# alasdairforsythe/tokenmonster

Hardware: AMD Instinct MI355X
Metric: GB/s raw UTF-8 tokenized, englishcode-32000 vocab (higher is better)
Workload: dtype u8; 1 GPU; englishcode-32000-consistent vocabulary shape (synthetic, 32000 ids / 54181 index records), 1024 MiB raw synthetic mixed text per GPU in 300327 documents; end to end: input = RAW UTF-8 resident in HBM, normalized (NFD+capcode) on the GPU inside the timed step, output = uint32 ids + offsets in HBM; raw_bytes_per_gpu=1073743404, normalized_bytes_per_gpu=1145560274, missing=0, parallelism=documents sharded by rank, no collective, rccl_ranks=0

## Files before the change

tokenmonster_amd/csrc/tm_norm.hip:

```cpp
#include <hip/hip_runtime.h>

#include <algorithm>
#include <chrono>
#include <cstring>
#include <mutex>
#include <thread>
#include <vector>

#include "tm_pipeline.h"
#include "tm_build.h"
#include "tm_norm_masks.h"

using namespace tmh;

namespace tmh {

constexpr int PIECE = 1024, PMARGIN = 68, PLDS = PIECE + 2 * PMARGIN;
constexpr uint32_t PS_WHOLE = 1u, PS_LEADU_SHIFT = 1, PS_LEADTL = 8u, PS_TRAILU_SHIFT = 5, PS_FIRSTBLOCK = 128u, PS_FIRSTL = 256u, PS_BAD = 512u;

__device__ __forceinline__ uint32_t ncls_ascii(uint32_t c, bool lower_all) {
  if (c - 'a' < 26u) return NC_L;
  if (c - 'A' < 26u) return lower_all ? NC_L : NC_U;
  if (c - '0' < 10u) return NC_N;
  if (c == '\'') return NC_AP;
// ... 232 lines not shown
  if (np_dev) npieces = min(npieces, np_dev[0]);
  __shared__ PieceLds s_l[4];
  __shared__ uint8_t s_cls[128];
  __shared__ TabLds s_tab;
  if (threadIdx.x < 128) s_cls[threadIdx.x] = (uint8_t)ncls_ascii(threadIdx.x, lower_all != 0);
  const NmTabs tabs = stage_tabs(s_tab, two);
  __syncthreads();
  const int lane = threadIdx.x & 63, wv = threadIdx.x >> 6;
  const uint64_t k = (uint64_t)blockIdx.x * 4 + wv;
  if (k >= npieces) return;
  PieceLds& L = s_l[wv];
  const uint32_t d = piece_doc[k];
  if (MODE != 3 && need_host[d]) { if (MODE != 1 && lane == 0) piece_len[k] = 0; return; }
  const uint64_t rb = rbegin[d], re = rend[d], pb = rb + (k - doc_piece_start[d]) * PIECE;
  const int m = norm_load_piece(L, raw, rb, re, pb, lane, s_cls, &s_tab, two);
  uint8_t* dst = MODE == 1 ? out + piece_off[k] : (MODE >= 2 ? out + k * (uint64_t)SLAB : nullptr);
  if (capcode != 2 || MODE == 3) {
    if (MODE != 1 && lane == 0) piece_len[k] = (uint32_t)m;
    bool bad = false;
    if (WRITE) for (int i = lane; i < m; i += 64) {
      const int x = PMARGIN + i;
      if (MODE == 3) bad |= L.f[x] == NF_BAD;
      uint32_t b = L.raw[x], y = 0, m3 = 0;
      if (lower_all && b - 'A' < 26u) b |= 0x20u;
      const uint32_t bm1 = L.raw[x - 1];
      if (nm_two_lead(b)) (void)nm_two_out(nm_two_get(tabs, nm_two_index(b, L.raw[x + 1])), false, false, false, &b, &y, &m3);
      else if (nm_cont_byte(b) && nm_two_lead(bm1)) (void)nm_two_out(nm_two_get(tabs, nm_two_index(bm1, b)), true, false, false, &b, &y, &m3);
      dst[i] = (uint8_t)b;
    }
    if (MODE == 3 && __any(bad) && lane == 0) need_host[d] = 1;
    return;
  }
  const uint32_t carry = piece_carry[k];
  const unsigned long long below = (1ull << lane) - 1ull;
  {
    uint32_t carry_ua = (carry >> 2) & 3u;
    bool carry_tl = (carry >> 4) & 1u;
    for (int c = (m - 1) / 64; c >= 0; c--) {
      const int i = c * 64 + lane;
      const bool in = i < m;
      const uint32_t fl = in ? L.f[PMARGIN + i] : 0u, cls = fl & NF_CLASS;
      const unsigned long long V = __ballot(in), mB = __ballot(in && nblock(cls)), mU = __ballot(in && cls == NC_U), mL = __ballot(in && cls == NC_L);
      const unsigned long long above = lane == 63 ? 0ull : (~0ull << (lane + 1));
      const unsigned long long stop = V & ~mB & above;
      uint32_t ua;
      bool tl;
      if (stop != 0) {
        const int e = __ffsll((long long)stop) - 1;
        ua = (uint32_t)__popcll(mU & above & ((1ull << e) - 1ull));
        tl = (mL >> e) & 1ull;
      } else {
        ua = (uint32_t)__popcll(mU & above) + carry_ua;
        tl = carry_tl;
      }
      ua = min(ua, 2u);
      if (in && nblock(cls)) L.f[PMARGIN + i] = (uint8_t)(fl | (tl ? NF_TERML : 0u) | (ua << NF_UA_SHIFT));
      const uint32_t ua0 = __shfl(ua, 0), cls0 = __shfl(cls, 0);
      const bool tl0 = __shfl((int)tl, 0) != 0;
      if (nblock(cls0)) { carry_ua = min(ua0 + (cls0 == NC_U ? 1u : 0u), 2u); carry_tl = tl0; }
      else { carry_ua = 0; carry_tl = cls0 == NC_L; }
    }
  }
  const bool next_tl = (carry >> 4) & 1u;
  __builtin_amdgcn_wave_barrier();
  __builtin_amdgcn_s_waitcnt(0);
  uint32_t carry_ub = carry & 3u;
  uint32_t pos = 0;
  for (int c = 0; c * 64 < m; c++) {
    const int i = c * 64 + lane, x = PMARGIN + i;
    const bool in = i < m;
    const uint32_t fl = in ? L.f[x] : 0u, cls = fl & NF_CLASS;
    const unsigned long long mB = __ballot(in && nblock(cls)), mU = __ballot(in && cls == NC_U);
    const unsigned long long gap = ~mB & below;
    uint32_t ub;
    if (gap != 0) {
      const int s = 64 - __clzll((long long)gap);
      ub = (uint32_t)__popcll(mU & below & ~((1ull << s) - 1ull));
    } else ub = (uint32_t)__popcll(mU & below) + carry_ub;
    ub = min(ub, 2u);
    {
      const uint32_t ub63 = __shfl(ub, 63), cls63 = __shfl(cls, 63);
      carry_ub = nblock(cls63) ? min(ub63 + (cls63 == NC_U ? 1u : 0u), 2u) : 0u;
    }
    uint32_t o0 = 0, o1 = 0, o2 = 0, o3 = 0, len = 0;
    if (in) {
      const uint32_t b = L.raw[x];
      const uint32_t fm1 = L.f[x - 1], P = fm1 & NF_CLASS;
      uint32_t P2 = NC_O;
      if (P == NC_AP) P2 = L.f[(fm1 & NF_CONT) ? x - 4 : x - 2] & NF_CLASS;
      const bool inword = ub >= 1;
      const bool tl = (fl & NF_TERML) != 0;
      const uint32_t code = nm_lut_entry(nm_lut_index((fl & NF_CONT) ? (uint32_t)NC_O : cls, P, P2, inword ? 1u : 0u, tl ? 1u : 0u), lower_all != 0);
      len = (code & 3u) + 1u;
      o0 = 'D'; o1 = code >> 8; o2 = ' ';
      o3 = b | ((code & 4u) << 3);
      if (cls == NC_SP) {
        const bool last = i + 1 == m;
        const uint32_t fp1 = L.f[x + 1];
        if ((fp1 & NF_CLASS) == NC_U && fp1 != NF_BAD && !(fp1 & NF_CONT)) o3 = (last ? next_tl : (fp1 & NF_TERML) != 0) ? 'C' : 'W';
      }
      const uint32_t bm1 = L.raw[x - 1];
      const bool lead2 = nm_two_lead(b), cont2 = nm_cont_byte(b) && nm_two_lead(bm1);
      if (lead2 || cont2) {
        const NmTwo e = nm_two_get(tabs, lead2 ? nm_two_index(b, L.raw[x + 1]) : nm_two_index(bm1, b));
        uint32_t y = 0, m3 = 0;
        const uint32_t extra = nm_two_out(e, cont2, (code & 4u) != 0, true, &o3, &y, &m3);
        if (extra >= 1u) { len = 1u + extra; o2 = y; o1 = m3; }
      }
      uint32_t hrole, hcp;
      if ((tabs.misc & NM_MISC_HANGUL) && fl != NF_BAD && nm_hangul_role(b, bm1, L.raw[x - 2], L.raw[x + 1], L.raw[x + 2], &hrole, &hcp)) len = nm_hangul_out(hcp, hrole, &o1, &o2, &o3);
      uint32_t lrole, lidx;
      if ((tabs.misc & NM_MISC_LEA) && fl != NF_BAD && nm_lea_role(b, bm1, L.raw[x - 2], L.raw[x + 1], L.raw[x + 2], &lrole, &lidx) && (tabs.lea[lidx].a & NT_OK)) {
        const NmLea le = tabs.lea[lidx];
        if (lrole == 0u) o3 = (code & 4u) ? ((le.a >> 16) & 0xFFu) : ((le.a >> 8) & 0xFFu);
        else if (lrole == 1u) { len = 2u; o2 = le.b & 0xFFu; o3 = (le.b >> 8) & 0xFFu; }
        else if (((le.a >> 24) & 3u) == 2u) { len = 2u; o2 = (le.b >> 16) & 0xFFu; o3 = le.b >> 24; }
        else len = 0u;
      }
      uint32_t krole, kidx;
      if ((tabs.misc & NM_MISC_KANA) && fl != NF_BAD && nm_kana_role(b, bm1, L.raw[x - 2], L.raw[x + 1], L.raw[x + 2], &krole, &kidx) && (nm_kana_tab(tabs)[kidx] & NK_OK))
        len = nm_kana_out(nm_kana_tab(tabs)[kidx], krole, &o1, &o2, &o3);
      uint32_t drole, dcp;
      if ((tabs.misc & NM_MISC_DEC3) && fl != NF_BAD && nm_three_role(b, bm1, L.raw[x - 2], L.raw[x + 1], L.raw[x + 2], &drole, &dcp) && (nm_dec3(tabs, dcp) & ND_OK))
        len = nm_dec3_out(tabs, nm_dec3(tabs, dcp), drole, &o1, &o2, &o3);
    }
    uint32_t incl = len;
#pragma unroll
    for (uint32_t q = 1; q <= 4; q++) {
      const unsigned long long bq = __ballot(len >= q);
      incl = __builtin_amdgcn_mbcnt_hi((uint32_t)(bq >> 32), __builtin_amdgcn_mbcnt_lo((uint32_t)bq, incl));
    }
    if (WRITE && in && (MODE == 1 || pos + incl <= (uint32_t)SLAB)) {
      uint8_t* w = dst + pos + (incl - len);
      if (len == 4) { w[0] = (uint8_t)o0; w[1] = (uint8_t)o1; w[2] = (uint8_t)o2; w[3] = (uint8_t)o3; }
      else if (len == 3) { w[0] = (uint8_t)o1; w[1] = (uint8_t)o2; w[2] = (uint8_t)o3; }
      else if (len == 2) { w[0] = (uint8_t)o2; w[1] = (uint8_t)o3; }
      else if (len == 1) w[0] = (uint8_t)o3;
    }
    pos += __shfl(incl, 63);
  }
  if (MODE != 1 && lane == 0) {
    piece_len[k] = pos;
    if (MODE == 2 && pos > (uint32_t)SLAB) atomicAdd(overflow, 1ull);
  }
}

struct PieceLds2 { uint8_t raw[PLDS]; uint8_t f[PLDS]; uint8_t chg[32]; alignas(16) uint8_t out[2 * PIECE + 64]; };

__device__ const NmLut g_norm_lut = nm_make_lut();

#ifndef TM_NORM_UNROLL
#define TM_NORM_UNROLL 2
#endif
template <bool CARRY>
__global__ __launch_bounds__(256) void k_norm_emit2(const uint8_t* __restrict__ raw, const uint64_t* __restrict__ rbegin,
                                                    const uint64_t* __restrict__ rend, const uint32_t* __restrict__ piece_doc,
                                                    const uint64_t* __restrict__ doc_piece_start, uint64_t npieces, uint32_t lower_all,
                                                    const uint8_t* __restrict__ piece_carry, uint8_t* __restrict__ need_host,
                                                    uint32_t* __restrict__ piece_len, uint8_t* __restrict__ slab,
                                                    unsigned long long* __restrict__ overflow, const NmTwo* __restrict__ two,
                                                    const uint64_t* __restrict__ np_dev) {
  constexpr int SLAB2 = 2 * PIECE, NCH = PIECE / 64;
  if (np_dev) npieces = min(npieces, np_dev[0]);
  __shared__ PieceLds2 s_l[4];
  __shared__ uint8_t s_cls[128];
  __shared__ TabLds s_tab;
  const NmTabs tabs = stage_tabs(s_tab, two);
  alignas(16) __shared__ uint16_t s_lut[NM_LUT_SIZE];
  static_assert(NM_LUT_SIZE * sizeof(uint16_t) == 256 * sizeof(uint4), "one 16-byte load per thread stages the rule table");
  if (threadIdx.x < 128) s_cls[threadIdx.x] = (uint8_t)ncls_ascii(threadIdx.x, lower_all != 0);
  reinterpret_cast<uint4*>(s_lut)[threadIdx.x] = reinterpret_cast<const uint4*>(g_norm_lut.e[lower_all ? 1 : 0])[threadIdx.x];
  __syncthreads();
  const int lane = threadIdx.x & 63, wv = __builtin_amdgcn_readfirstlane((int)(threadIdx.x >> 6));
  PieceLds2& L = s_l[wv];
#pragma unroll 1
  for (uint64_t k = (uint64_t)blockIdx.x * 4 + wv; k < npieces; k += (uint64_t)gridDim.x * 4) {
  const uint32_t d = piece_doc[k];
  if (CARRY && need_host[d]) { if (lane == 0) piece_len[k] = 0; continue; }
  const uint64_t rb = rbegin[d], re = rend[d], pb = rb + (k - doc_piece_start[d]) * PIECE;
  const int m = __builtin_amdgcn_readfirstlane(norm_load_piece(L, raw, rb, re, pb, lane, s_cls, &s_tab, two));
  const uint32_t carry = CARRY ? __builtin_amdgcn_readfirstlane((uint32_t)piece_carry[k]) : 0u;
  const int nch = (m + 63) >> 6;
  const uint8_t* fl0 = L.f + PMARGIN + lane;
  unsigned long long w_seed = (carry & 3u) ? 1ull : 0ull;
  const unsigned long long t0_beyond = CARRY ? (unsigned long long)((carry >> 4) & 1u) : 0ull;
  if (!CARRY) {
    const uint32_t fb = fl0[-64], fa = m == PIECE ? (uint32_t)fl0[64 * NCH] : 0u;
    uint64_t w_in;
    const bool known = nm_margin_carries(__ballot((fb & NF_BLOCK) != 0), __ballot((fb & NF_CLASS) == NC_U), __ballot((fa & NF_BLOCK) != 0), &w_in);
    if (!known && lane == 0) atomicAdd(overflow + 1, 1ull);
    w_seed = w_in;
  }
  typedef TM_LDS_SPACE uint8_t lds_u8;
  const uint32_t out0 = TM_LDS_ADDR(L.out);
  const uint32_t dump = out0 + (uint32_t)SLAB2 + (uint32_t)lane;
  const uint32_t lim = out0 + (uint32_t)SLAB2;
  unsigned long long w = w_seed, badm = 0ull;
  uint32_t posabs = out0;
  bool over = false;
  uint32_t chC = 'C', chW = 'W', chSP = ' ', chD = 'D';
  TM_KEEP_IN_VGPRS4(chC, chW, chSP, chD);
  const uint8_t* fc = fl0;
  const uint8_t* rc = L.raw + PMARGIN + lane;
  uint32_t fl = fc[0];
  unsigned long long Bcur = __ballot((fl & NF_BLOCK) != 0), Lcur = __ballot((fl & NF_CLASS) == NC_L), Ucur = __ballot((fl & NF_CLASS) == NC_U);
  int c = 0;
  auto chunk = [&]() __attribute__((always_inline)) {
    const uint32_t fnext = fc[64];
    const unsigned long long Bn = __ballot((fnext & NF_BLOCK) != 0), Ln = __ballot((fnext & NF_CLASS) == NC_L), Un = __ballot((fnext & NF_CLASS) == NC_U);
    unsigned long long t0n = Ln >> __builtin_ctzll(~Bn | (1ull << 63));
    if (__builtin_expect(Bn == ~0ull, 0)) {
      t0n = t0_beyond;
#pragma unroll 1
      for (int j = c + 2; j <= NCH; j++) {
        const uint32_t fj = fl0[64 * j];
        const unsigned long long Bj = __ballot((fj & NF_BLOCK) != 0), Lj = __ballot((fj & NF_CLASS) == NC_L);
        if (Bj != ~0ull) { t0n = nm_t0(Bj, Lj, 0ull); break; }
      }
    }
    const unsigned long long TXc = nm_tx(Bcur, Lcur, t0n);
    const uint32_t fp = fc[-1], f2 = fc[-2], f4 = fc[-4];
    const uint32_t b = rc[0];
    uint64_t w_out, spC, spW;
    if (!CARRY) badm |= __ballot(fl == NF_BAD);
    const unsigned long long W = nm_inword(Bcur, Ucur, ~0ull, w, &w_out);
    nm_space_markers(__ballot((fl & NF_CLASS) == NC_SP), Ucur, Un, ~0ull, TXc, t0n, &spC, &spW);
    w = w_out;
    const uint32_t p2 = (fp & NF_CONT) ? f4 : f2;
    uint32_t idx = ((fl & NF_CONT) ? (uint32_t)NC_O : (fl & 7u)) | ((fp & 7u) << 3) | ((p2 & 7u) << 6);
    idx = sel_mask(W, idx | 512u, idx);
    idx = sel_mask(TXc, idx | 1024u, idx);
    const uint32_t code = s_lut[idx];
    uint32_t len1 = code & 3u;
    uint32_t o3 = b | ((code & 4u) << 3);
    o3 = sel_mask(spC, chC, o3);
    o3 = sel_mask(spW, chW, o3);
    uint32_t ysp = chSP, m3 = code >> 8;
    unsigned long long E = ~0ull;
    uint32_t below = posabs + (uint32_t)lane, n = len1 + 1u;
    if (__ballot(b >= 0x80u) != 0ull && __builtin_amdgcn_readfirstlane((int)L.chg[c]) != 0) {
      if (b >= 0x80u) {
        const HighOut h = emit_high_byte(rc, fl, code, HighOut{o3, ysp, m3, len1}, &s_tab, two);
        o3 = h.o3; ysp = h.ysp; m3 = h.m3; len1 = h.len1;
      }
      E = ~__ballot(len1 == 0xFFu);
      len1 = len1 == 0xFFu ? 0u : len1;
      n = sel_mask(E, len1 + 1u, 0u);
      below = mbcnt64(E, posabs);
    }
    const unsigned long long ge2 = __ballot(len1 >= 1u), ge3 = __ballot(len1 >= 2u), ge4 = __ballot(len1 >= 3u);
    const uint32_t first = mbcnt64(ge4, mbcnt64(ge3, mbcnt64(ge2, below)));
    const uint32_t last = first + len1;
    const uint32_t end = read_lane(first + n, 63);
    if (end <= lim) {
      *TM_LDS_PTR(lds_u8, sel_mask(E, last, dump)) = (uint8_t)o3;
      *TM_LDS_PTR(lds_u8, sel_mask(ge2, last - 1u, dump)) = (uint8_t)ysp;
      *TM_LDS_PTR(lds_u8, sel_mask(ge3, last - 2u, dump)) = (uint8_t)m3;
      *TM_LDS_PTR(lds_u8, sel_mask(ge4, first, dump)) = (uint8_t)chD;
    } else over = true;
    posabs = end;
    fl = fnext; Bcur = Bn; Lcur = Ln; Ucur = Un;
    c++; fc += 64; rc += 64;
  };
#pragma unroll 1
  while (c + TM_NORM_UNROLL <= nch) {
#pragma unroll
    for (int u = 0; u < TM_NORM_UNROLL; u++) chunk();
  }
#pragma unroll 1
  while (c < nch) chunk();
  const uint32_t pos = posabs - out0 - (uint32_t)(64 * nch - m);
  __builtin_amdgcn_wave_barrier();
  __builtin_amdgcn_s_waitcnt(0);
  if (!over) {
    uint8_t* dst = slab + k * (uint64_t)SLAB2;
    for (uint32_t j = (uint32_t)lane * 16u; j < pos; j += 64u * 16u)
      *reinterpret_cast<uint4*>(dst + j) = *reinterpret_cast<const uint4*>(L.out + j);
  }
  if (lane == 0) {
    piece_len[k] = pos;
    if (over) atomicAdd(overflow, 1ull);
    if (!CARRY && badm != 0ull) need_host[d] = 1;
  }
  __builtin_amdgcn_wave_barrier();
  }
}


__global__ void k_norm_begin(const uint64_t* __restrict__ rbegin, const uint64_t* __restrict__ rend, uint32_t ndocs, uint32_t* __restrict__ doc_npiece, uint8_t* __restrict__ need_host,
                             unsigned long long* __restrict__ ninfo) {
  const uint32_t d = blockIdx.x * blockDim.x + threadIdx.x;
  if (d < 8) ninfo[d] = 0ull;
  if (d < ndocs) {
    doc_npiece[d] = (uint32_t)((rend[d] - rbegin[d] + PIECE - 1) / PIECE);
    need_host[d] = 0;
  }
}

__global__ void k_norm_bad(const uint32_t* __restrict__ piece_doc, const uint8_t* __restrict__ need_host, const uint64_t* __restrict__ doc_piece_start, uint64_t npieces,
                           uint32_t ndocs, uint32_t* __restrict__ piece_len, unsigned long long* __restrict__ ninfo, uint32_t* __restrict__ fb_ids,
                           const uint64_t* __restrict__ np_dev) {
  const uint64_t k = (uint64_t)blockIdx.x * blockDim.x + threadIdx.x;
  if (np_dev && k >= np_dev[0]) { if (k < npieces) piece_len[k] = 0; }
  else if (k < npieces) {
    const uint32_t d = piece_doc[k];
    if (need_host[d]) piece_len[k] = 0;
    else if (piece_len[k] < (uint32_t)TEXT_LEN && k + 1 != doc_piece_start[d + 1]) atomicAdd(&ninfo[6], 1ull);
  }
  if (k < ndocs && need_host[k]) fb_ids[atomicAdd(&ninfo[0], 1ull)] = (uint32_t)k;
}

__global__ void k_norm_short(const uint32_t* __restrict__ piece_doc, const uint8_t* __restrict__ need_host, const uint64_t* __restrict__ doc_piece_start, uint64_t npieces,
                             const uint32_t* __restrict__ piece_len, unsigned long long* __restrict__ ninfo) {
  const uint64_t k = (uint64_t)blockIdx.x * blockDim.x + threadIdx.x;
  if (k >= npieces) return;
  const uint32_t d = piece_doc[k];
  if (!need_host[d] && piece_len[k] < (uint32_t)TEXT_LEN && k + 1 != doc_piece_start[d + 1]) atomicAdd(&ninfo[6], 1ull);
}

__global__ __launch_bounds__(256) void k_norm_compact(const uint8_t* __restrict__ slab, const uint32_t* __restrict__ piece_len,
                                                      const uint64_t* __restrict__ piece_off, uint64_t npieces, uint8_t* __restrict__ out, uint64_t cap) {
  const int lane = threadIdx.x & 63;
  const uint64_t k = (uint64_t)blockIdx.x * 4 + (threadIdx.x >> 6);
  if (k >= npieces) return;
  const uint32_t len = piece_len[k];
  if (piece_off[k] + len > cap) return;
  const uint8_t* src = slab + k * (uint64_t)SLAB;
  uint8_t* dst = out + piece_off[k];
  for (uint32_t i = (uint32_t)lane * 16u; i < len; i += 64u * 16u) {
    if (i + 16u <= len) { uint4 q; __builtin_memcpy(&q, src + i, 16); __builtin_memcpy(dst + i, &q, 16); }
    else for (uint32_t j = i; j < len; j++) dst[j] = src[j];
  }
}

__global__ void k_norm_ranges(const uint64_t* __restrict__ piece_off, const uint64_t* __restrict__ doc_piece_start, const uint8_t* __restrict__ need_host,
                              uint32_t ndocs, uint64_t* __restrict__ nbegin, uint64_t* __restrict__ nend) {
  const uint32_t d = blockIdx.x * blockDim.x + threadIdx.x;
  if (d >= ndocs) return;
  if (need_host[d]) return;
  nbegin[d] = piece_off[doc_piece_start[d]];
  nend[d] = piece_off[doc_piece_start[d + 1]];
}
__global__ void k_norm_ranges_info(const uint64_t* __restrict__ piece_off, const uint64_t* __restrict__ doc_piece_start, const uint8_t* __restrict__ need_host,
                                   uint32_t ndocs, uint64_t* __restrict__ nbegin, uint64_t* __restrict__ nend, unsigned long long* __restrict__ ninfo, uint32_t long_segs) {
  const uint32_t d = blockIdx.x * blockDim.x + threadIdx.x;
  uint64_t nseg = 0;
  if (d < ndocs && !need_host[d]) {
    const uint64_t a = piece_off[doc_piece_start[d]], b = piece_off[doc_piece_start[d + 1]];
    nbegin[d] = a; nend[d] = b;
    nseg = (b - a + SEG - 1) / SEG;
    if (nseg > long_segs) atomicAdd(&ninfo[1], 1ull);
  }
  for (int o = 32; o > 0; o >>= 1) nseg += __shfl_xor(nseg, o);
  if ((threadIdx.x & 63) == 0 && nseg) atomicAdd(&ninfo[2], (unsigned long long)nseg);
}
__global__ void k_norm_info(const uint64_t* __restrict__ nbegin, const uint64_t* __restrict__ nend, uint32_t ndocs, unsigned long long* __restrict__ ninfo,
                            uint32_t long_segs) {
  const uint32_t d = blockIdx.x * blockDim.x + threadIdx.x;
  uint64_t nseg = 0;
  if (d < ndocs) { nseg = (nend[d] - nbegin[d] + SEG - 1) / SEG; if (nseg > long_segs) atomicAdd(&ninfo[1], 1ull); }
  for (int o = 32; o > 0; o >>= 1) nseg += __shfl_xor(nseg, o);
  if ((threadIdx.x & 63) == 0 && nseg) atomicAdd(&ninfo[2], (unsigned long long)nseg);
}
constexpr uint32_t PF_NONE = 0xFFFFFFFFu;
#ifndef TM_PF_SPAN
#define TM_PF_SPAN 4096u
#endif
#ifndef TM_PF_WHOLE
#define TM_PF_WHOLE 16384u
#endif
constexpr uint32_t PF_SPAN = TM_PF_SPAN, PF_WHOLE = TM_PF_WHOLE, PF_GAP = 32u;
static_assert(PF_SPAN % 256u == 0u && PF_SPAN >= (uint32_t)PIECE && PF_WHOLE >= PF_SPAN, "a span is whole steps of the sweep, and the spans' table lives in the pieces' arrays");
__host__ __device__ __forceinline__ uint32_t pf_spans(uint64_t n) { return n <= PF_WHOLE ? (n ? 1u : 0u) : (uint32_t)((n + PF_SPAN - 1) / PF_SPAN); }
struct PfPiece { uint32_t s1, s2, fq, a, z; };
struct PfDoc { uint32_t s1, s2, qb, a, z, zlo; };
__host__ __device__ __forceinline__ uint64_t pf_out_begin(uint64_t raw_begin, uint32_t d) { return ((raw_begin + 15ull) & ~15ull) + (uint64_t)PF_GAP * d; }
__device__ __forceinline__ bool pf_isq(uint32_t y) { return y == 0x98u || y == 0x99u || y == 0x9Cu || y == 0x9Du; }
__device__ __forceinline__ uint32_t pf_eq(uint32_t v, uint32_t c4) { const uint32_t t = v ^ c4; return ~(((t & 0x7F7F7F7Fu) + 0x7F7F7F7Fu) | t) & 0x80808080u; }
__device__ __forceinline__ uint32_t pf_isq4(uint32_t v) { return pf_eq(v & 0xFAFAFAFAu, 0x98989898u); }
__device__ __forceinline__ uint32_t pf_nb4(uint32_t v) { return (((v & 0x7F7F7F7Fu) + 0x5F5F5F5Fu) | v) & 0x80808080u; }
__device__ __forceinline__ uint32_t pf_load(const TmWindow& win, uint32_t off, uint32_t n) {
  uint32_t v = tm_window_u32(win, off);
  const uint32_t rem = n - off;
  if (rem < 4u) v &= (1u << (8u * rem)) - 1u;
  return v;
}
__device__ __forceinline__ uint32_t pf_first(unsigned long long any, uint32_t m, uint32_t base) {
  const int l = __builtin_ctzll(any);
  return base + 4u * (uint32_t)l + ((uint32_t)__builtin_ctz(read_lane(m, l)) >> 3);
}
__device__ __forceinline__ uint32_t pf_last(unsigned long long any, uint32_t m, uint32_t base) {
  const int l = 63 - __builtin_clzll(any);
  return base + 4u * (uint32_t)l + ((31u - (uint32_t)__builtin_clz(read_lane(m, l))) >> 3);
}
__device__ __forceinline__ bool pf_suppressed(uint32_t flags, const PfDoc& d, uint32_t t) {
  return (flags & 16u) && d.s1 < t && t < d.s2 && d.qb == 0u;
}
__device__ __forceinline__ PfPiece pf_scan_span(const TmWindow& win, uint32_t n, uint32_t rb, uint32_t re, uint32_t flags, bool whole, uint32_t lane) {
  PfPiece r{PF_NONE, PF_NONE, PF_NONE, PF_NONE, PF_NONE};
  const bool fused = (flags & 16u) && (flags & 128u), trim = flags & 32u;
  bool want_s = (flags & 8u) && (flags & 16u), want_a = trim;
  uint32_t carry = rb >= 4u ? pf_load(win, rb - 4u, n) : 0u;
#pragma unroll 1
  for (uint32_t base = rb; base < re && (want_s || want_a); base += 256u) {
    const uint32_t x = pf_load(win, base + 4u * lane, n);
    const uint32_t pd = TM_DPP(carry, x, 0x138, 0xF);
    carry = read_lane(x, 63);
    if (want_s) {
      const uint32_t p1 = (x << 8) | (pd >> 24), p2 = (x << 16) | (pd >> 16);
      uint32_t S = pf_eq(x, 0x20202020u) & pf_eq(p1, 0x20202020u);
      if (fused) S |= pf_eq(x, 0x0A0A0A0Au) & pf_eq(p1, 0x0D0D0D0Du);
      const uint32_t Q = pf_isq4(x) & pf_eq(p1, 0x80808080u) & pf_eq(p2, 0xE2E2E2E2u);
      unsigned long long mS = __ballot(S != 0u);
      while (mS != 0ull && r.s2 == PF_NONE) {
        const int l = __builtin_ctzll(mS);
        uint32_t m = read_lane(S, l);
        const uint32_t pos = base + 4u * (uint32_t)l + ((uint32_t)__builtin_ctz(m) >> 3);
        if (r.s1 == PF_NONE) r.s1 = pos; else r.s2 = pos;
        m &= m - 1u;
        if ((int)lane == l) S = m;
        if (m == 0u) mS &= mS - 1ull;
      }
      const unsigned long long mQ = __ballot(Q != 0u);
// ... 714 lines not shown
```

tokenmonster_amd/csrc/tm_norm_masks.h:

```cpp
#pragma once
#include <cstdint>

#if defined(__HIP__)
#define TM_HD __host__ __device__ inline __attribute__((always_inline))
#else
#define TM_HD inline
#endif

namespace tmh {

enum : uint32_t { NC_O = 0, NC_L = 1, NC_SP = 2, NC_LO = 3, NC_U = 4, NC_N = 5, NC_AP = 6, NC_M = 7 };
constexpr uint32_t NF_CLASS = 7u, NF_BLOCK = 4u, NF_CONT = 8u, NF_TERML = 16u, NF_UA_SHIFT = 5, NF_BAD = 0x80u;

struct NmTwo { uint32_t a, b; };
constexpr int NM_TWO_LEADS = 30, NM_TWO_SIZE = NM_TWO_LEADS * 64, NM_TWO_FAST = 256;
constexpr uint32_t NT_OK = 8u, NT_DECOMP = 16u, NT_DECOMP2 = 32u;
TM_HD bool nm_two_lead(uint32_t b) { return b - 0xC2u < (uint32_t)NM_TWO_LEADS; }
TM_HD bool nm_three_lead(uint32_t b) { return (b & 0xF0u) == 0xE0u; }
TM_HD bool nm_cont_byte(uint32_t b) { return (b & 0xC0u) == 0x80u; }
TM_HD uint32_t nm_two_index(uint32_t lead, uint32_t second) { return ((lead - 0xC2u) << 6) | (second & 63u); }
TM_HD bool nm_punct3(uint32_t b1, uint32_t b2) {
  return (b1 == 0x80u && ((b2 >= 0x90u && b2 <= 0xA7u) || (b2 >= 0xB0u && b2 <= 0xBFu))) || (b1 == 0x81u && b2 >= 0x80u && b2 <= 0x9Eu);
}
constexpr int NM_BLK_WORDS = 64, NM_CP_WORDS = 4096;
// ... 73 lines not shown
  if (!nm_cont_byte(b1) || !nm_cont_byte(b2)) return false;
  *cp = nm_cp3(lead, b1, b2);
  return true;
}
TM_HD uint32_t nm_dec3_out(const NmTabs& t, uint32_t e, uint32_t role, uint32_t* o1, uint32_t* o2, uint32_t* o3) {
  if (role == 2u && ((e >> 26) & 15u) == 0u) return 0u;
  const uint32_t cp = role == 2u ? nm_dec3_last(t, e) : 0x800u + ((role == 0u ? e : e >> 13) & 0x1FFFu);
  *o1 = 0xE0u | (cp >> 12); *o2 = 0x80u | ((cp >> 6) & 63u); *o3 = 0x80u | (cp & 63u);
  return 3u;
}
TM_HD uint32_t nm_ccc3(const NmTabs& t, uint32_t cp) { return ((t.misc & NM_MISC_CCC) && cp - NM_CCC_BASE < NM_CCC_SIZE) ? (uint32_t)nm_ccc_tab(t)[cp - NM_CCC_BASE] : 0u; }
TM_HD NmTwo nm_two_get(const NmTabs& t, uint32_t idx) { return idx < (uint32_t)NM_TWO_FAST ? t.two_fast[idx] : t.two_all[idx]; }
TM_HD uint32_t nm_three_code(const NmTabs& t, uint32_t cp) {
  const uint32_t bc = (t.blk[cp >> 10] >> (2u * ((cp >> 6) & 15u))) & 3u;
  return bc != 3u ? bc : ((t.cp[cp >> 4] >> (2u * (cp & 15u))) & 3u);
}
TM_HD uint32_t nm_four_code(const NmTabs& t, uint32_t lead, uint32_t b1, uint32_t b2, uint32_t b3) {
  if (!nm_cont_byte(b1) || !nm_cont_byte(b2) || !nm_cont_byte(b3)) return 0u;
  const uint32_t cp = ((lead & 7u) << 18) | ((b1 & 63u) << 12) | ((b2 & 63u) << 6) | (b3 & 63u);
  if (cp - 0x10000u >= 0x100000u) return 0u;
  const uint32_t blk = (cp - 0x10000u) >> 6;
  const uint32_t code = (t.blk4[blk >> 4] >> (2u * (blk & 15u))) & 3u;
  return code == 3u ? 0u : code;
}
TM_HD uint32_t nm_classify_high(uint32_t b, uint32_t m1, uint32_t m2, uint32_t m3, uint32_t p1, uint32_t p2, uint32_t p3, const NmTabs& tabs) {
  if (nm_two_lead(b)) {
    if (!nm_cont_byte(p1)) return NF_BAD;
    const uint32_t a = nm_two_get(tabs, nm_two_index(b, p1)).a;
    if (!(a & NT_OK)) return NF_BAD;
    if ((a & NF_CLASS) == NC_M && nm_cont_byte(m1) && nm_two_lead(m2)) {
      const uint32_t pa = nm_two_get(tabs, nm_two_index(m2, m1)).a;
      if ((pa & NF_CLASS) == NC_M || (pa & (NT_DECOMP | NT_DECOMP2))) return NF_BAD;
    }
    if ((a & NF_CLASS) == NC_M && (tabs.misc & NM_MISC_LEA) && m3 == 0xE1u && m2 - 0xB8u < 4u && nm_cont_byte(m1) && (tabs.lea[((m2 & 3u) << 6) | (m1 & 63u)].a & NT_OK)) return NF_BAD;
    if ((a & NF_CLASS) == NC_M && nm_three_lead(m3) && nm_cont_byte(m2) && nm_cont_byte(m1) && nm_ccc3(tabs, nm_cp3(m3, m2, m1)) - 1u < NM_CCC_LOWER - 1u) return NF_BAD;
    if ((a & NF_CLASS) == NC_M && nm_three_lead(m3) && nm_cont_byte(m2) && nm_cont_byte(m1)) {
      const uint32_t pe = nm_dec3(tabs, nm_cp3(m3, m2, m1));
      if ((pe & ND_OK) && nm_ccc3(tabs, nm_dec3_last(tabs, pe)) - 1u < NM_CCC_LOWER - 1u) return NF_BAD;
    }
    if ((a & NF_CLASS) == NC_M && (tabs.misc & NM_MISC_KANA) && m3 == 0xE3u && m2 - 0x81u < 3u && nm_cont_byte(m1) && (nm_kana_tab(tabs)[((m2 - 0x81u) << 6) | (m1 & 63u)] & NK_OK)) return NF_BAD;
    return a & NF_CLASS;
  }
  if (nm_cont_byte(b) && nm_two_lead(m1)) {
    const uint32_t a = nm_two_get(tabs, nm_two_index(m1, b)).a;
    return (a & NT_OK) ? ((a & (NT_DECOMP | NT_DECOMP2)) ? (uint32_t)NC_M : ((a & NF_CLASS) | NF_CONT)) : NF_BAD;
  }
  uint32_t lead = 0, b1 = 0, b2 = 0, cont = 0;
  if (nm_three_lead(b)) { lead = b; b1 = p1; b2 = p2; }
  else if (nm_cont_byte(b) && nm_three_lead(m1)) { lead = m1; b1 = b; b2 = p1; cont = NF_CONT; }
  else if (nm_cont_byte(b) && nm_cont_byte(m1) && nm_three_lead(m2)) { lead = m2; b1 = m1; b2 = b; cont = NF_CONT; }
  else {
    uint32_t code = 0u;
    if (nm_four_lead(b)) code = nm_four_code(tabs, b, p1, p2, p3);
    else if (nm_cont_byte(b)) {
      cont = NF_CONT;
      if (nm_four_lead(m1)) code = nm_four_code(tabs, m1, b, p1, p2);
      else if (nm_four_lead(m2)) code = nm_four_code(tabs, m2, m1, b, p1);
      else if (nm_four_lead(m3)) code = nm_four_code(tabs, m3, m2, m1, b);
    }
    return code == 0u ? (uint32_t)NF_BAD : ((code == 2u ? (uint32_t)NC_LO : (uint32_t)NC_O) | cont);
  }
  if (!nm_cont_byte(b1) || !nm_cont_byte(b2)) return NF_BAD;
  if (lead == 0xE2u && nm_punct3(b1, b2)) return ((b1 == 0x80u && b2 == 0x99u) ? (uint32_t)NC_AP : (uint32_t)NC_O) | cont;
  const uint32_t cp3 = nm_cp3(lead, b1, b2);
  if ((tabs.misc & NM_MISC_LEA) && cp3 - 0x1E00u < (uint32_t)NM_LEA_SIZE) {
    const uint32_t a = tabs.lea[cp3 - 0x1E00u].a;
    if (a & NT_OK) return cont ? (uint32_t)NC_M : (a & NF_CLASS);
  }
  if ((tabs.misc & NM_MISC_KANA) && cp3 - 0x3040u < (uint32_t)NM_KANA_SIZE && (nm_kana_tab(tabs)[cp3 - 0x3040u] & NK_OK)) return cont ? (uint32_t)NC_M : (uint32_t)NC_LO;
  { const uint32_t de = nm_dec3(tabs, cp3);
    if (de & ND_OK) return cont ? (uint32_t)NC_M : ((de & ND_LETTER) ? (uint32_t)NC_LO : (uint32_t)NC_M); }
  const uint32_t code = nm_three_code(tabs, cp3);
  if (code == 0u) {
    const uint32_t c = nm_ccc3(tabs, cp3);
    if (c == NM_CCC_DIGIT) return (uint32_t)NC_N | cont;
    if (c == NM_CCC_LOWER) return (uint32_t)NC_L | cont;
    if (c != 0u) {
      if (!cont) {
        if (nm_cont_byte(m1) && nm_two_lead(m2)) {
          const uint32_t pa = nm_two_get(tabs, nm_two_index(m2, m1)).a;
          if ((pa & NF_CLASS) == NC_M || (pa & (NT_DECOMP | NT_DECOMP2))) return NF_BAD;
        } else if (nm_cont_byte(m1) && nm_cont_byte(m2) && nm_three_lead(m3)) {
          const uint32_t pcp = nm_cp3(m3, m2, m1);
          const uint32_t pe = nm_dec3(tabs, pcp);
          const uint32_t pc = nm_ccc3(tabs, (pe & ND_OK) ? nm_dec3_last(tabs, pe) : pcp);
          if (pc < NM_CCC_LOWER && pc > c) return NF_BAD;
          if ((tabs.misc & NM_MISC_LEA) && pcp - 0x1E00u < (uint32_t)NM_LEA_SIZE && (tabs.lea[pcp - 0x1E00u].a & NT_OK)) return NF_BAD;
          if ((tabs.misc & NM_MISC_KANA) && pcp - 0x3040u < (uint32_t)NM_KANA_SIZE && (nm_kana_tab(tabs)[pcp - 0x3040u] & NK_OK)) return NF_BAD;
        }
      }
      return (uint32_t)NC_M | cont;
    }
  }
  if (code == 0u && (tabs.misc & NM_MISC_HANGUL) && nm_hangul(cp3)) return (uint32_t)NC_LO | cont;
  return code == 0u ? (uint32_t)NF_BAD : ((code == 3u ? (uint32_t)NC_M : (code == 2u ? (uint32_t)NC_LO : (uint32_t)NC_O)) | cont);
}
TM_HD uint32_t nm_classify_char(uint32_t b, uint32_t m1, uint32_t m2, uint32_t m3, uint32_t p1, uint32_t p2, uint32_t p3, const NmTabs& tabs) {
  const uint32_t cls = nm_classify_high(b, m1, m2, m3, p1, p2, p3, tabs);
  if (cls == NF_BAD || !(nm_two_lead(b) || nm_three_lead(b) || nm_four_lead(b))) return NF_BAD | (NF_BAD << 8) | (1u << 16);
  uint32_t cont = cls | NF_CONT, n = 4u, changes = 0u;
  if (nm_two_lead(b)) {
    n = 2u; changes = 1u;
    if (nm_two_get(tabs, nm_two_index(b, p1)).a & (NT_DECOMP | NT_DECOMP2)) cont = NC_M;
  } else if (nm_three_lead(b)) {
    n = 3u;
    const uint32_t cp3 = nm_cp3(b, p1, p2);
    if (((tabs.misc & NM_MISC_LEA) && cp3 - 0x1E00u < (uint32_t)NM_LEA_SIZE && (tabs.lea[cp3 - 0x1E00u].a & NT_OK)) ||
        ((tabs.misc & NM_MISC_KANA) && cp3 - 0x3040u < (uint32_t)NM_KANA_SIZE && (nm_kana_tab(tabs)[cp3 - 0x3040u] & NK_OK)) || (nm_dec3(tabs, cp3) & ND_OK)) { cont = NC_M; changes = 1u; }
    else if ((tabs.misc & NM_MISC_HANGUL) && nm_hangul(cp3)) changes = 1u;
  }
  return cls | (cont << 8) | (n << 16) | (changes << 24);
}
TM_HD uint32_t nm_two_out(NmTwo e, bool cont, bool lowered, bool capcode, uint32_t* o3, uint32_t* y, uint32_t* m3) {
  if (!cont) { *o3 = lowered ? (e.b & 0xFFu) : ((e.a >> 8) & 0xFFu); return 0u; }
  const bool upper = capcode && (e.a & NF_CLASS) == NC_U;
  if (e.a & NT_DECOMP) { *y = (e.a >> 16) & 0xFFu; *o3 = e.a >> 24; return 1u; }
  if (e.a & NT_DECOMP2) { *m3 = upper ? ((e.b >> 8) & 0xFFu) : ((e.a >> 16) & 0xFFu); *y = e.a >> 24; *o3 = (e.b >> 16) & 0xFFu; return 2u; }
  *o3 = upper ? ((e.b >> 8) & 0xFFu) : ((e.a >> 16) & 0xFFu);
  return 0u;
}

TM_HD uint64_t nm_brev(uint64_t x) { return __builtin_bitreverse64(x); }
TM_HD uint64_t nm_flood_up(uint64_t M, uint64_t S) { S &= M; return ((M ^ (M + S)) | S) & M; }
TM_HD uint64_t nm_flood_down_inside(uint64_t M, uint64_t S) { const uint64_t m = nm_brev(M), s = nm_brev(S); return nm_brev(((m ^ (m + s)) | s) & m); }
TM_HD uint64_t nm_shr1(uint64_t cur, uint64_t next0) { return (cur >> 1) | (next0 << 63); }
TM_HD uint64_t nm_valid(int c, int m) { const int r = m - 64 * c; return r >= 64 ? ~0ull : (r <= 0 ? 0ull : ((1ull << r) - 1ull)); }

TM_HD uint64_t nm_t0(uint64_t B, uint64_t L, uint64_t beyond) {
  const uint64_t nb = ~B;
  return nb == 0ull ? (beyond & 1ull) : ((L >> __builtin_ctzll(nb)) & 1ull);
}
TM_HD uint64_t nm_tx(uint64_t B, uint64_t L, uint64_t t0_next) { return nm_flood_down_inside(B, B & nm_shr1(L, t0_next & 1ull)); }

TM_HD uint64_t nm_inword(uint64_t B, uint64_t U, uint64_t V, uint64_t w_in, uint64_t* w_out) {
  const uint64_t G = nm_flood_up(B & V, (U & V) | (w_in & 1ull));
  *w_out = G >> 63;
  return (G << 1) | (w_in & 1ull);
}

TM_HD void nm_space_markers(uint64_t SP, uint64_t U, uint64_t next_u0, uint64_t V, uint64_t tx, uint64_t tx_next0, uint64_t* spC, uint64_t* spW) {
  const uint64_t spM = SP & V & nm_shr1(U, next_u0 & 1ull);
  const uint64_t nextT = nm_shr1(tx, tx_next0 & 1ull);
  *spC = spM & nextT;
  *spW = spM & ~nextT;
}

TM_HD bool nm_margin_carries(uint64_t Bb, uint64_t Ub, uint64_t Ba, uint64_t* w_in) {
  uint64_t w_out;
  (void)nm_inword(Bb, Ub, ~0ull, 0ull, &w_out);
  *w_in = w_out;
  return !((Bb == ~0ull && Ub == 0ull) || Ba == ~0ull);
}

constexpr int NM_LUT_SIZE = 2048;
TM_HD constexpr uint32_t nm_lut_index(uint32_t cls, uint32_t prev, uint32_t prev2, uint32_t w, uint32_t t) {
  return (cls & 7u) | ((prev & 7u) << 3) | ((prev2 & 7u) << 6) | ((w & 1u) << 9) | ((t & 1u) << 10);
}
TM_HD constexpr uint16_t nm_lut_entry(uint32_t idx, bool lower_all) {
  const uint32_t cls = idx & 7u, P = (idx >> 3) & 7u, P2 = (idx >> 6) & 7u;
  const bool W = (idx >> 9) & 1u, T = (idx >> 10) & 1u;
  const bool Pletter = P == NC_L || P == NC_U || P == NC_LO, P2letter = P2 == NC_L || P2 == NC_U || P2 == NC_LO;
  uint32_t len = 1, lower = 0, mark = 0;
  if (cls == NC_U) {
    lower = 1;
    if (!W) {
      if (P == NC_SP) len = 2;
      else { len = 4; mark = T ? 'C' : 'W'; }
    } else if (T) { len = 4; mark = 'C'; }
    else if (P == NC_N) { len = 3; mark = 'D'; }
  } else if (cls == NC_L) {
    lower = lower_all ? 1 : 0;
    const bool joined = W ? (P == NC_U || P == NC_AP || P == NC_M)
                          : (P == NC_SP || Pletter || P == NC_M || (P == NC_AP && P2letter));
    if (!joined) { len = 3; mark = 'D'; }
  } else if (cls == NC_N) {
    const bool joined = W ? (P == NC_N) : (P == NC_SP || P == NC_N);
    if (!joined) { len = 3; mark = 'D'; }
  }
  return (uint16_t)((len - 1) | (lower << 2) | (mark << 8));
}
struct NmLut { uint16_t e[2][NM_LUT_SIZE]; };
constexpr NmLut nm_make_lut() {
  NmLut t{};
  for (int la = 0; la < 2; la++)
    for (int i = 0; i < NM_LUT_SIZE; i++) t.e[la][i] = nm_lut_entry((uint32_t)i, la != 0);
  return t;
}

}
```

Baseline: 47.43 GB/s.

## Add packed four-chunk ASCII fast path to normalization emit kernel

In the non-carry normalization kernel, adds a group4 path that handles four 64-byte chunks at once when they are all ASCII. Each lane packs four bytes into one 32-bit word, and the word-state scan and output-length prefix sum run as packed DPP scans. The per-chunk path remains as a fallback for high bytes, fully blocked chunks, or slab overflow. This is meant to cut the per-chunk ballot and scan overhead in the common ASCII case, at the cost of more code, more register pressure, and a second implementation of the same logic that must stay consistent with the first. It also changes the overflow check to account for the tail padding on the last chunk.

```diff
diff --git a/tokenmonster_amd/csrc/tm_norm.hip b/tokenmonster_amd/csrc/tm_norm.hip
--- a/tokenmonster_amd/csrc/tm_norm.hip
+++ b/tokenmonster_amd/csrc/tm_norm.hip
@@ -408,6 +408,19 @@
 #ifndef TM_NORM_UNROLL
 #define TM_NORM_UNROLL 2
 #endif
+__device__ __forceinline__ void norm_scan_pairs(uint32_t& s, uint32_t& q) {
+#define TM_NM_ROW(ctrl) { const uint32_t ts = TM_DPP0(s, ctrl), tq = TM_DPP0(q, ctrl); nm4_combine(&s, &q, ts, tq); }
+#define TM_NM_BC(ctrl, rows) { const uint32_t ts = TM_DPP(0u, s, ctrl, rows), tq = TM_DPP(0u, q, ctrl, rows); nm4_combine(&s, &q, ts, tq); }
+  TM_NM_ROW(0x111) TM_NM_ROW(0x112) TM_NM_ROW(0x114) TM_NM_ROW(0x118)
+  TM_NM_BC(0x142, 0xA) TM_NM_BC(0x143, 0xC)
+#undef TM_NM_ROW
+#undef TM_NM_BC
+}
+__device__ __forceinline__ uint32_t norm_scan_add(uint32_t x) {
+  x += TM_DPP0(x, 0x111); x += TM_DPP0(x, 0x112); x += TM_DPP0(x, 0x114); x += TM_DPP0(x, 0x118);
+  x += TM_DPP(0u, x, 0x142, 0xA); x += TM_DPP(0u, x, 0x143, 0xC);
+  return x;
+}
 template <bool CARRY>
 __global__ __launch_bounds__(256) void k_norm_emit2(const uint8_t* __restrict__ raw, const uint64_t* __restrict__ rbegin,
                                                     const uint64_t* __restrict__ rend, const uint32_t* __restrict__ piece_doc,
@@ -508,7 +521,7 @@
     const uint32_t first = mbcnt64(ge4, mbcnt64(ge3, mbcnt64(ge2, below)));
     const uint32_t last = first + len1;
     const uint32_t end = read_lane(first + n, 63);
-    if (end <= lim) {
+    if (end - (c + 1 == nch ? (uint32_t)(64 * nch - m) : 0u) <= lim) {
       *TM_LDS_PTR(lds_u8, sel_mask(E, last, dump)) = (uint8_t)o3;
       *TM_LDS_PTR(lds_u8, sel_mask(ge2, last - 1u, dump)) = (uint8_t)ysp;
       *TM_LDS_PTR(lds_u8, sel_mask(ge3, last - 2u, dump)) = (uint8_t)m3;
@@ -518,13 +531,74 @@
     fl = fnext; Bcur = Bn; Lcur = Ln; Ucur = Un;
     c++; fc += 64; rc += 64;
   };
+  const uint32_t lane2 = (uint32_t)lane * 0x00010001u, rev4 = (63u - (uint32_t)lane) * 4u;
+  auto group4 = [&]() __attribute__((always_inline)) -> bool {
+    const uint32_t b0 = rc[0], b1 = rc[64], b2 = rc[128], b3 = rc[192];
+    if (__ballot(((b0 | b1 | b2 | b3 | (uint32_t)rc[-2]) & 0x80u) != 0u) != 0ull) return false;
+    const uint32_t fnext = fc[256];
+    const unsigned long long Bn = __ballot((fnext & NF_BLOCK) != 0), Ln = __ballot((fnext & NF_CLASS) == NC_L), Un = __ballot((fnext & NF_CLASS) == NC_U);
+    if (__builtin_expect(Bn == ~0ull, 0)) return false;
+    const uint32_t t0n = (uint32_t)(Ln >> __builtin_ctzll(~Bn)) & 1u;
+    const uint32_t F = fl | ((uint32_t)fc[64] << 8) | ((uint32_t)fc[128] << 16) | ((uint32_t)fc[192] << 24);
+    const uint32_t raw4 = b0 | (b1 << 8) | (b2 << 16) | (b3 << 24);
+    const uint32_t Fp = TM_DPP((read_lane(F, 63) << 8) | (uint32_t)fc[-1], F, 0x138, 0xF);
+    const uint32_t F2 = TM_DPP((read_lane(F, 62) << 8) | (uint32_t)fc[-2], Fp, 0x138, 0xF);
+    const Nm4Cls cl = nm4_classes(F);
+    uint32_t s, q;
+    nm4_pairs(cl, (uint32_t)__builtin_amdgcn_ds_bpermute((int)rev4, (int)nm4_rev_in(cl)), &s, &q);
+    norm_scan_pairs(s, q);
+    uint32_t w_out;
+    const uint32_t cin = nm4_chain(read_lane(s, 63), read_lane(q, 63), (uint32_t)w, t0n, &w_out);
+    const uint32_t G = nm4_fill(s, q, cin);
+    const uint32_t wtu = nm4_wtu(cl, TM_DPP(cin, G, 0x138, 0xF), (uint32_t)__builtin_amdgcn_ds_bpermute((int)rev4, (int)G));
+    const uint32_t behind = TM_DPP(nm4_behind63(read_lane(wtu, 0), (uint32_t)Un, t0n), wtu, 0x130, 0xF);
+    const uint32_t o3 = nm4_out3(raw4, cl, behind);
+    const uint32_t ie = nm4_index2(F, Fp, F2, wtu, 0u), io = nm4_index2(F, Fp, F2, wtu, 1u);
+    const uint32_t c02 = (uint32_t)s_lut[ie & 0xFFFFu] | ((uint32_t)s_lut[ie >> 16] << 16), c13 = (uint32_t)s_lut[io & 0xFFFFu] | ((uint32_t)s_lut[io >> 16] << 16);
+    const uint32_t le = c02 & 0x00030003u, lo = c13 & 0x00030003u, len4 = le | (lo << 8);
+    const uint32_t inc = norm_scan_add(len4), ex = inc - len4, tot = read_lane(inc, 63);
+    const uint32_t p0 = posabs - out0, p1 = p0 + 64u + (tot & 255u), p2 = p1 + 64u + ((tot >> 8) & 255u), p3 = p2 + 64u + ((tot >> 16) & 255u), pe = p3 + 64u + (tot >> 24);
+    if (pe - (c + 4 == nch ? (uint32_t)(64 * nch - m) : 0u) > (uint32_t)SLAB2) return false;
+    const uint32_t fe = (ex & NM4_H) + (p0 | (p2 << 16)) + lane2, fo = ((ex >> 8) & NM4_H) + (p1 | (p3 << 16)) + lane2;
+    const uint32_t one = 0x00010001u;
+    const uint32_t a4e = fe + le, a3e = fe + le - ((le | (le >> 1)) & one), a2e = fe + (le & (le >> 1));
+    const uint32_t a4o = fo + lo, a3o = fo + lo - ((lo | (lo >> 1)) & one), a2o = fo + (lo & (lo >> 1));
+#define TM_NM_PUT(A1, A2, A3, A4, M3, O3) \
+    *TM_LDS_PTR(lds_u8, out0 + (A1)) = (uint8_t)chD; *TM_LDS_PTR(lds_u8, out0 + (A2)) = (uint8_t)(M3); \
+    *TM_LDS_PTR(lds_u8, out0 + (A3)) = (uint8_t)chSP; *TM_LDS_PTR(lds_u8, out0 + (A4)) = (uint8_t)(O3);
+    TM_NM_PUT(fe & 0xFFFFu, a2e & 0xFFFFu, a3e & 0xFFFFu, a4e & 0xFFFFu, c02 >> 8, o3)
+    TM_NM_PUT(fo & 0xFFFFu, a2o & 0xFFFFu, a3o & 0xFFFFu, a4o & 0xFFFFu, c13 >> 8, o3 >> 8)
+    TM_NM_PUT(fe >> 16, a2e >> 16, a3e >> 16, a4e >> 16, c02 >> 24, o3 >> 16)
+    TM_NM_PUT(fo >> 16, a2o >> 16, a3o >> 16, a4o >> 16, c13 >> 24, o3 >> 24)
+#undef TM_NM_PUT
+    posabs = out0 + pe;
+    w = w_out;
+    fl = fnext; Bcur = Bn; Lcur = Ln; Ucur = Un;
+    c += 4; fc += 256; rc += 256;
+    return true;
+  };
+  if (CARRY) {
 #pragma unroll 1
-  while (c + TM_NORM_UNROLL <= nch) {
+    while (c + TM_NORM_UNROLL <= nch) {
 #pragma unroll
-    for (int u = 0; u < TM_NORM_UNROLL; u++) chunk();
-  }
+      for (int u = 0; u < TM_NORM_UNROLL; u++) chunk();
+    }
 #pragma unroll 1
-  while (c < nch) chunk();
+    while (c < nch) chunk();
+  } else {
+#pragma unroll 1
+    while (c < nch) {
+      if (!over && c + 4 <= nch && group4()) continue;
+      const int ce = c + 4 < nch ? c + 4 : nch;
+#pragma unroll 1
+      while (c + TM_NORM_UNROLL <= ce) {
+#pragma unroll
+        for (int u = 0; u < TM_NORM_UNROLL; u++) chunk();
+      }
+#pragma unroll 1
+      while (c < ce) chunk();
+    }
+  }
   const uint32_t pos = posabs - out0 - (uint32_t)(64 * nch - m);
   __builtin_amdgcn_wave_barrier();
   __builtin_amdgcn_s_waitcnt(0);
diff --git a/tokenmonster_amd/csrc/tm_norm_masks.h b/tokenmonster_amd/csrc/tm_norm_masks.h
--- a/tokenmonster_amd/csrc/tm_norm_masks.h
+++ b/tokenmonster_amd/csrc/tm_norm_masks.h
@@ -249,6 +249,40 @@
   return !((Bb == ~0ull && Ub == 0ull) || Ba == ~0ull);
 }
 
+constexpr uint32_t NM4_LO = 0x01010101u, NM4_H = 0x00FF00FFu;
+struct Nm4Cls { uint32_t B, U, L, SP; };
+TM_HD Nm4Cls nm4_classes(uint32_t F) {
+  const uint32_t b0 = F, b1 = F >> 1, b2 = F >> 2;
+  return Nm4Cls{b2 & NM4_LO, b2 & ~b1 & ~b0 & NM4_LO, b0 & ~b1 & ~b2 & NM4_LO, b1 & ~b0 & ~b2 & NM4_LO};
+}
+TM_HD uint32_t nm4_rev_in(const Nm4Cls& k) { return k.L | ((k.B ^ NM4_LO) << 1); }
+TM_HD void nm4_pairs(const Nm4Cls& k, uint32_t rev, uint32_t* s, uint32_t* q) {
+  *s = k.U | ((rev & NM4_LO) << 1);
+  *q = (k.B ^ NM4_LO) | (rev & (NM4_LO << 1));
+}
+TM_HD void nm4_combine(uint32_t* s, uint32_t* q, uint32_t ts, uint32_t tq) { *s |= ts & ~*q; *q |= tq; }
+TM_HD uint32_t nm4_chain(uint32_t S, uint32_t Q, uint32_t w_in, uint32_t x_in, uint32_t* w_out) {
+  uint32_t cin = 0u, w = w_in & 1u, x = x_in & 1u;
+  for (uint32_t u = 0; u < 4u; u++) { cin |= w << (8u * u); w = ((S >> (8u * u)) | (w & ~(Q >> (8u * u)))) & 1u; }
+  for (uint32_t u = 4u; u-- > 0u;) { cin |= x << (8u * u + 1u); x = ((S >> (8u * u + 1u)) | (x & ~(Q >> (8u * u + 1u)))) & 1u; }
+  *w_out = w;
+  return cin;
+}
+TM_HD uint32_t nm4_fill(uint32_t s, uint32_t q, uint32_t cin) { return s | (cin & ~q); }
+TM_HD uint32_t nm4_wtu(const Nm4Cls& k, uint32_t g_before, uint32_t x) { return (g_before & NM4_LO) | (x & (k.B << 1)) | (k.U << 2); }
+TM_HD uint32_t nm4_behind63(uint32_t wtu_lane0, uint32_t next_u0, uint32_t next_t0) { return (wtu_lane0 >> 8) | ((((next_u0 & 1u) << 2) | ((next_t0 & 1u) << 1)) << 24); }
+TM_HD uint32_t nm4_space_c(const Nm4Cls& k, uint32_t behind) { return k.SP & (behind >> 2) & (behind >> 1); }
+TM_HD uint32_t nm4_space_w(const Nm4Cls& k, uint32_t behind) { return k.SP & (behind >> 2) & ~(behind >> 1); }
+TM_HD uint32_t nm4_out3(uint32_t raw, const Nm4Cls& k, uint32_t behind) {
+  const uint32_t spm = (k.SP & (behind >> 2)) * 0xFFu;
+  const uint32_t mk = 0x57575757u - ((behind >> 1) & NM4_LO) * 0x14u;
+  return ((raw | ((k.U | k.L) << 5)) & ~spm) | (mk & spm);
+}
+TM_HD uint32_t nm4_index2(uint32_t F, uint32_t Fp, uint32_t F2, uint32_t wtu, uint32_t odd) {
+  const uint32_t sh = 8u * odd;
+  return ((F >> sh) & NM4_H) | (((Fp >> sh) & NM4_H) << 3) | (((F2 >> sh) & NM4_H) << 6) | (((wtu >> sh) & 0x00030003u) << 9);
+}
+
 constexpr int NM_LUT_SIZE = 2048;
 TM_HD constexpr uint32_t nm_lut_index(uint32_t cls, uint32_t prev, uint32_t prev2, uint32_t w, uint32_t t) {
   return (cls & 7u) | ((prev & 7u) << 3) | ((prev2 & 7u) << 6) | ((w & 1u) << 9) | ((t & 1u) << 10);
```

Result: faster. 48.18 GB/s, median of 6 (+1.6%).
